# BriansIDP/espnet_slurp

Measured on AMD Instinct MI355X. Metric: utterances/sec (fbank80x1500, Conformer-12L CTC+attn), higher is better.
Workload: dtype f32; 1 GPU; C2 SLURP Conformer-medium d=256 H=4 FF=1024 12L enc / 6L dec, V=600, rel_pos=latest, ctc 0.3, lsm 0.1, dropout 0.1, SpecAug on; global_batch=384, seq_len=1500, parallelism=dp1

## Files before the change

espnet_slurp_amd/_native.py:

```python
from __future__ import annotations

import ctypes
import os

_HERE = os.path.dirname(os.path.abspath(__file__))
LIB_PATH = os.path.join(_HERE, "libespnet_mi355%s.so" % os.environ.get("ESP_LIB_VARIANT", ""))

P = ctypes.c_void_p
I = ctypes.c_int
L = ctypes.c_long
F = ctypes.c_float
U64 = ctypes.c_ulonglong

SIGNATURES = {
    "esp_last_error": [],
    "esp_abi_version": [],
    "esp_gemm_bf16": [I, I, I, I, I, I, I, P, L, L, L, P, L, L, L, P, L, L, L, P, F, F, P, I, P, F, U64, I, P, P, P, L,
                      P],
    "esp_gemm_bf16_pl": [I, I, I, I, I, I, I, P, L, L, L, P, L, L, L, P, L, L, L, P, F, F, I, P, F, U64, I, P, I,
                         L, P, L, P],
    "esp_f32_to_bf16": [P, P, L, I, L, L, I, P],
    "esp_conv2_fwd_bf16": [P, P, P, P, I, I, I, I, P, L, P],
    "esp_conv2_dgrad_bf16": [P, P, P, P, I, I, I, I, P, P, L, P],
    "esp_conv1_fwd_bf16": [P, P, P, P, P, I, I, I, I, P],
    "esp_conv2_wgrad_bf16": [P, P, P, P, I, I, I, I, P, L, P],
    "esp_gemm_f32": [I, I, I, I, I, I, I, P, L, L, L, P, L, L, L, P, L, L, L, P, F, F, P, I, P, F, U64, I, P, P,
                     P, P, P, L, P],
    "esp_gemm_f32_bp": [I, I, I, I, I, I, I, P, L, L, L, P, L, L, L, P, L, L, L, P, F, F, P, I, P, F, U64, I, P, P,
                        P, P, L, P, L, L, L, L, P],
    "esp_f32_to_planes": [P, P, L, I, L, L, L, P],
    "esp_gemm_f32_pl": [I, I, I, I, I, I, I, P, L, L, L, P, L, L, L, L, P, L, L, L, P, L, L, L, L, P, L, L, L, P, F, F,
                        P, I, P, F, U64, I, P, P, I, L, P, L, P],
    "esp_set_gemm_compute": [I],
    "esp_get_gemm_compute": [],
    "esp_f32_gemm_products": [],
    "esp_set_splitk_mode": [I],
    "esp_set_wgrad_ws": [I],
    "esp_set_fwd_ws": [I],
    "esp_get_fwd_ws_launches": [],
    "esp_act_bwd": [P, P, P, L, I, F, U64, L, P],
    "esp_scale_dropout": [P, P, L, F, F, U64, P, F, P],
    "esp_scale_dropout_planes": [P, P, L, L, I, F, F, U64, P],
    "esp_scale_by_dev": [P, L, P, P],
    "esp_embed_fwd": [P, P, P, P, I, I, I, F, F, U64, P],
    "esp_embed_bwd": [P, P, P, I, I, I, F, F, U64, P],
    "esp_specaug": [P, P, I, I, I, P, P, P, I, P, I, P],
    "esp_utterance_mvn": [P, I, I, I, P, P],
    "esp_grad_norm": [P, L, F, P, L, P, P],
    "esp_adam": [P, P, P, P, L, P, F, ctypes.c_double, ctypes.c_double, F, F, I, P],
    "esp_opt_hyper": [P, ctypes.c_double, ctypes.c_double, ctypes.c_double, ctypes.c_double, P, P],
    "esp_adam_dev": [P, P, P, P, L, P, P, ctypes.c_double, ctypes.c_double, F, F, P],
    "esp_adam_amsgrad": [P, P, P, P, P, L, P, F, ctypes.c_double, ctypes.c_double, F, F, I, P],
    "esp_adam_dev_amsgrad": [P, P, P, P, P, L, P, P, ctypes.c_double, ctypes.c_double, F, F, P],
    "esp_opt_advance": [P, P, P],
# ... 95 lines not shown
    "esp_layernorm_bwd_workspace_bytes": [I, I],
    "esp_colsum_workspace_bytes": [I, I],
    "esp_dwconv1d_wgrad_workspace_bytes": [I, I, I, I],
    "esp_ebf_merge_bwd_workspace_bytes": [I, I, I, I],
    "esp_bn_swish_fwd_workspace_bytes": [I, I],
    "esp_bn_swish_bwd_workspace_bytes": [I, I],
    "esp_conv1_wgrad_workspace_bytes": [I, I, I, I],
    "esp_conv2_dgrad_workspace_bytes": [I],
    "esp_ctc_loss_workspace_bytes": [I, I, I],
    "esp_rnnt_joint_bwd_workspace_bytes": [I, I, I, I],
    "esp_rnnt_loss_workspace_bytes": [I, I, I],
    "esp_relpos_dp_workspace_bytes": [I, I, I],
}
_RESTYPES = {"esp_last_error": ctypes.c_char_p, "esp_abi_version": I, "esp_attn_slot_check_errors": I, "esp_set_gemm_compute": I,
             "esp_get_gemm_compute": I, "esp_set_splitk_mode": I, "esp_set_wgrad_ws": I, "esp_set_fwd_ws": I, "esp_get_fwd_ws_launches": L,
             "esp_f32_gemm_products": I}
_RESTYPES.update({k: L for k in SIGNATURES if k.endswith("_workspace_bytes")})
ABI_VERSION = 42

_lib = None


def load() -> ctypes.CDLL:
    global _lib
    if _lib is not None:
        return _lib
    if not os.path.exists(LIB_PATH):
        raise RuntimeError(
            f"espnet_slurp_amd: native library not found at {LIB_PATH}; "
            "build it with `make -C espnet_slurp_amd/csrc` (no CPU fallback exists)")
# ... 31 lines not shown
```

espnet_slurp_amd/csrc/gemm.hip:

```cpp
#include <stdlib.h>

#include <algorithm>

#include "gemm_kernels.h"

using namespace espg;

namespace {

bool aligned16(const void* p) { return ((uintptr_t)p & 15) == 0; }

constexpr int RED_SLOTS = 64, RED_GROUPS = 4;
__global__ __launch_bounds__(256) void splitk_reduce4_kernel(GemmArgs g) {
  __shared__ float4 part[RED_GROUPS][RED_SLOTS];
  const long MN = (long)g.M * g.N;
  const long split_stride = MN * g.batch;
  if (g.rowsum && g.rs_work) {
    const long m = blockIdx.x * (long)blockDim.x + threadIdx.x;
    if (m < g.M) {
      float acc = 0.f;
      int s = 0;
      for (; s + 8 <= g.splits; s += 8) {
        float v[8];
#pragma unroll
// ... 71 lines not shown
  out[r] += s;
}

long g_cus = -1;
long persist_blocks(int per_cu) {
  if (g_cus < 0) {
    int dev = 0, cus = 256;
    if (hipGetDevice(&dev) == hipSuccess)
      if (hipDeviceGetAttribute(&cus, hipDeviceAttributeMultiprocessorCount, dev) != hipSuccess) cus = 256;
    g_cus = cus;
  }
  return (long)per_cu * g_cus;
}

int g_compute = 0;
int g_last_grid = 0;

int g_splitk = 0;
int splitk_mode() { return g_splitk; }

int g_wgrad_ws = 1;
int g_fwd_ws = 1;
long g_fwd_ws_launches = 0;

constexpr long kSplitkMinK = 256;
long splitk_mink() { return kSplitkMinK; }

constexpr long kSplitkTarget = 2 * 256;
constexpr long kMaxSplits = 128;
#ifndef ESP_GEMM_TILE_TIE
#define ESP_GEMM_TILE_TIE 0.95
#endif

bool launch_glds(int MA, int MB, const GemmArgs& g, int batch, hipStream_t st, const GldsArgs* tconv = nullptr) {
  const int BNT = g.bnt;
  const bool can_rs = MA == RC;
  const bool can_fwd = (MA == KC && (MB == KC || MB == RC)) || (MA == I2C_KC && MB == KC);
  const bool can_bwd = (MA == KC || MA == I2CT_KC) && MB == RC;
  const bool can_spec_fwd = MA == KC && MB == KC, can_spec_bwd = MA == KC && MB == RC;
  const bool can_brelu = (MA == KC || MA == I2C_KC) && MB == KC;
  const bool can_pspec = (MA == KC || MA == RC) && (MB == KC || MB == RC);
  if (MA == I2C_KC && (g.a.ic.C % GL_BK || g.K % GL_BK)) return false;
  if (MA == I2C_KC && 8L * g.a.ic.H * g.a.ic.W * g.a.ic.C >= (1L << 32)) return false;
  if (MB == I2C_RC) {
    const long kpix = g.bf16 == 2 ? 2L * g.K : (long)g.K;
    if (!i2c_rc_off24_ok(g.b.ic, kpix)) return false;
  }
  int kind = g.splits > 1 ? EPI_PLAIN : epi_kind_spec(g);
  if (g.cpn) {
// ... 15 lines not shown
  const int bm = g.bm == 64 || g.bm == 256 ? g.bm : BM;
  x.nty = (g.M + bm - 1) / bm;
  if (MA == I2C_KC) {
    x.c_a = make_fastdiv(g.a.ic.C);
    x.hw_a = make_fastdiv(g.a.ic.Ho * g.a.ic.Wo);
    x.wo_a = make_fastdiv(g.a.ic.Wo);
  }
  if (MB == I2C_RC) {
    x.c_b = make_fastdiv(g.b.ic.C);
    x.hw_b = make_fastdiv(g.b.ic.Ho * g.b.ic.Wo);
    x.wo_b = make_fastdiv(g.b.ic.Wo);
  }
  x.ntiles = (int)((long)x.ntx * x.nty * batch * g.splits);
  const bool rs = can_rs && g.rowsum;
  if (rs) kind = EPI_PLAIN;
  if (kind == EPI_C1FOLD && !(MA == I2CT_KC && MB == RC && BNT == 128 && bm == 128 && x.ntx <= C1NT)) return false;
  const dim3 grid((unsigned)std::min<long>(x.ntiles, persist_blocks(g.ws ? 1 : glds_occupancy_rt(BNT, kind, bm, g.bf16))));
  g_last_grid = (int)grid.x;
  x.fd_grid = make_fastdiv(grid.x);
  x.fd_ntx = make_fastdiv((uint32_t)x.ntx);
  x.fd_nty = make_fastdiv((uint32_t)x.nty);
  x.fd_splits = make_fastdiv((uint32_t)g.splits);
  x.fd_nb2 = make_fastdiv((uint32_t)g.nb2);
  const int prec = g.bf16;
  if (g.ws == 2) {
    if (rs || g.splits > 1 || MB != KC || !fwd_ws_launch(MA == I2C_KC, kind, grid, st, g, x)) return false;
    ++g_fwd_ws_launches;
    return true;
  }
  if (g.ws) return kind == EPI_PLAIN && wgrad_ws_launch(MB == I2C_RC, rs, grid, st, g, x);
  if (kind == EPI_PLAIN) return glds_launch_plain(MA, MB, BNT, prec, rs, grid, st, g, x);
  if (kind == EPI_FWD || kind == EPI_BWD) return glds_launch_epi(MA, MB, BNT, prec, kind, grid, st, g, x);
  if (kind == EPI_P0 || kind == EPI_PR || kind == EPI_SMB || kind == EPI_SMBN || kind == EPI_P0_PL)
    return glds_launch_pspec(MA, MB, BNT, prec, kind, grid, st, g, x);
  return glds_launch_spec(MA, MB, BNT, prec, kind, grid, st, g, x);
}

template <int MA, int MB>
int launch(const GemmArgs& g0, int batch, hipStream_t st, const Operand* b_fp32 = nullptr,
// ... 83 lines not shown
ESP_API int esp_f32_gemm_products(void) { return ESP_F32_SPLIT ? 6 : 1; }
ESP_API int esp_set_splitk_mode(int mode) {
  ESP_ARG_CHECK(mode == 0 || mode == 1, "esp_set_splitk_mode: mode must be 0 or 1, got %d", mode);
  const int prev = splitk_mode();
  g_splitk = mode;
  return prev;
}

ESP_API int esp_set_fwd_ws(int mode) {
  ESP_ARG_CHECK(mode >= 0 && mode <= 2, "esp_set_fwd_ws: mode must be 0, 1 or 2, got %d", mode);
  const int prev = g_fwd_ws;
  g_fwd_ws = mode;
  return prev;
}
ESP_API long esp_get_fwd_ws_launches(void) { return g_fwd_ws_launches; }

ESP_API int esp_set_wgrad_ws(int mode) {
  ESP_ARG_CHECK(mode >= 0 && mode <= 2, "esp_set_wgrad_ws: mode must be 0, 1 or 2, got %d", mode);
  const int prev = g_wgrad_ws;
  g_wgrad_ws = mode;
  return prev;
}

static int gemm_run(int mode_a, int mode_b, int M, int N, int K, int batch, int nb2, const float* A, long lda,
                    long sa1, long sa2, const float* B, long ldb, long sb1, long sb2, float* C, long ldc, long sc1,
                    long sc2, const float* bias, float alpha, float beta, const float* R, int act, float* aux,
                    float drop_p, unsigned long long seed, int bwd_act, const float* pre, float* rowsum,
                    const int* im2col_a, const int* im2col_b, float* work, long work_bytes, void* stream,
                    int prec_in, const GemmArgs* smb = nullptr, const void* b_planes = nullptr, long ldbp = 0,
                    long sbp1 = 0, long sbp2 = 0, long bps = 0, const void* a_planes = nullptr, long ldap = 0,
// ... 536 lines not shown
    hipLaunchKernelGGL(f32_to_planes_kernel, dim3((unsigned)std::min<long>((ps / 8 + 255) / 256, 8192)), dim3(256), 0,
                       st, wc_work, (uint4*)planes, 9L * D, D, (long)D, (long)D, ps, 1);
    ESP_CHECK_LAUNCH("esp_conv2_dgrad (planes)");
  }
  const int slot0[4] = {0, 4, 6, 8};
  C1Regions c1r{};
  long c1off = 0;
  for (int cls = 0; cls < 4; ++cls) {
    const int ph = cls >> 1, pw = cls & 1;
    const int Ha = (T1 - ph + 1) / 2, We = (F1 - pw + 1) / 2;
    const int nkt = ph ? 1 : 2, nkf = pw ? 1 : 2, ntap = nkt * nkf;
    GldsArgs t{};
    t.t_hw = make_fastdiv((uint32_t)(Ha * We));
    t.t_w = make_fastdiv((uint32_t)We);
    t.t_T2 = T2; t.t_F2 = F2; t.t_C = b16 ? D / 2 : D;
    for (int ti = 0; ti < ntap; ++ti) {
      const int kt = ph ? 1 : 2 * (ti / nkf), kf = pw ? 1 : 2 * (ti % nkf);
      t.t_dt[ti] = (kt - ph) / 2;
      t.t_df[ti] = (kf - pw) / 2;
    }
    t.t_zeros = zeros16;
    GemmArgs g{};
    g.M = B * Ha * We; g.N = D; g.K = b16 ? ntap * D / 2 : ntap * D; g.nb2 = 1;
    g.a = Operand{dz2, 0, 0, 0, 1, {}, 1};
    g.b = Operand{wc_work + (long)slot0[cls] * D * D, D, 0, 0, 1, {}, 1};
    g.c = dz1; g.ldc = D; g.alpha = 1.f; g.beta = 0.f;
    g.bwd_act = ACT_RELU; g.pre = z1bits ? zeros16 : z1;
    g.cm_bits = reinterpret_cast<const uint32_t*>(z1bits); g.cm_bw = D / 32;
    if (c1) {
      g.c = wc_work;
// ... 4 lines not shown
    if (bp) {
      g.b = Operand{reinterpret_cast<const float*>(planes + (long)slot0[cls] * D * D), D, 0, 0, 1, {}, 1};
      g.b.ps = ps;
      g.bf16 = 3;
    }
    if (b16) {
      g.b = Operand{reinterpret_cast<const float*>(planes + (long)slot0[cls] * D * D), D / 2, 0, 0, 1, {}, 1};
      g.bf16 = 2;
    }
    g.key = esp::rng_key_ptr();
    g.wide = 1;
    g.batch = 1; g.splits = 1; g.kchunk = g.K; g.bnt = D % 128 == 0 ? 128 : 64; g.bm = BM;
    g.cmap = 1;
    g.cm_hw = t.t_hw; g.cm_w = t.t_w;
    g.cm_T1 = T1; g.cm_F1 = F1; g.cm_ph = ph; g.cm_pw = pw;
    if (!launch_glds(I2CT_KC, RC, g, 1, st, &t)) {
      esp::set_error("esp_conv2_dgrad: no kernel for the class GEMM");
      return -1;
    }
    ESP_CHECK_LAUNCH("esp_conv2_dgrad");
    if (c1) {
      c1r.off[cls] = c1off;
      c1r.grid[cls] = g_last_grid;
      c1off += (long)g_last_grid * C1NT * 256 * 10;
    }
  }
  if (c1) {
    c1r.ncls = 4;
    float* red = c1->work + 4L * persist_blocks(4) * C1NT * 256 * 10;
    hipLaunchKernelGGL(c1fold_reduce_kernel, dim3((D / 128) * 4, C1_NCH), dim3(640), 0, st, c1->work, c1r, red);
    hipLaunchKernelGGL(c1fold_finalize_kernel, dim3((D * 10 + 255) / 256), dim3(256), 0, st, red, D, c1->dW, c1->db);
    ESP_CHECK_LAUNCH("esp_conv2_dgrad_c1fold (reduce)");
  }
  return 0;
}
```

espnet_slurp_amd/csrc/gemm_fwd_ws.hip:

```cpp
#include "gemm_kernels.h"

namespace espg {

#if ESP_FWD_WS && ESP_F32_SPLIT

namespace {

constexpr int FW_NT = 512;
constexpr int FW_PLA = FWD_WS_BM * 64, FW_PLB = FWD_WS_BN * 64;
constexpr int FW_STB = 3 * (FW_PLA + FW_PLB);

template <bool GA>
struct FwStageA {
  static constexpr int NI = FWD_WS_BM / 32;
  int rl, kq;
  uint32_t lds;
  __device__ __forceinline__ void init_lane(int pw, int lane) {
    const int qd = lane & 7;
    rl = 8 * pw + (lane >> 3);
    kq = 4 * qd;
    lds = (uint32_t)(rl * 64 + (((qd >> 1) ^ pl_kc_swz(rl)) << 4) + 8 * (qd & 1));
  }
  __device__ __forceinline__ long tap_off(const GemmArgs& g, const GldsArgs& x, int k0) const {
    const int t = (int)fdiv((uint32_t)k0, x.c_a), kt = t / 3, kf = t - 3 * kt;
    return ((long)kt * g.a.ic.W + kf) * g.a.ic.C + (k0 - t * g.a.ic.C);
  }
  __device__ __forceinline__ float4 load(const GemmArgs& g, const GldsArgs& x, int m0, int k0, long tap, int i) const {
    const int m = min(m0 + rl + 32 * i, g.M - 1);
    if constexpr (GA) {
      const float* p = g.a.p + tap + kq;
      return *reinterpret_cast<const float4*>(p + i2c_pix_off24(g.a.ic, x.hw_a, x.wo_a, (uint32_t)m));
    } else {
      return *reinterpret_cast<const float4*>(g.a.p + (long)m * g.a.ld + min(k0 + kq, g.K - 4));
    }
  }
  __device__ __forceinline__ void store(float4 w, int i, char* planes, int kv) const {
    if (!GA && kq >= kv) w = make_float4(0.f, 0.f, 0.f, 0.f);
    uint32_t h0, m0, l0, h1, m1, l1;
    esp::split3_pair<false>(w.x, w.y, h0, m0, l0);
    esp::split3_pair<false>(w.z, w.w, h1, m1, l1);
    char* d = planes + lds + i * 32 * 64;
    *reinterpret_cast<uint2*>(d) = make_uint2(h0, h1);
    *reinterpret_cast<uint2*>(d + FW_PLA) = make_uint2(m0, m1);
    *reinterpret_cast<uint2*>(d + 2 * FW_PLA) = make_uint2(l0, l1);
  }
};

template <bool GA, int EPI>
__global__ __launch_bounds__(FW_NT, 1) void gemm_fwd_ws_kernel(GemmArgs g, GldsArgs x) {
  constexpr int TM = 2, TN = 4;
  static_assert(2 * FW_STB <= 163840, "LDS");
  __shared__ __attribute__((aligned(16))) float smem[2 * FW_STB / 4];
  char* const sm = reinterpret_cast<char*>(smem);

  const int G = gridDim.x;
  int t = blockIdx.x;
  if (t >= x.ntiles) return;
  const int lane = threadIdx.x & 63;
  const int wave = __builtin_amdgcn_readfirstlane(threadIdx.x >> 6);
  const bool producer = wave >= 4;
  const int pw = wave & 3;
// ... 146 lines not shown
```

espnet_slurp_amd/csrc/gemm_kernels.h:

```cpp
#pragma once
#include <stdlib.h>

#include <algorithm>

#include <type_traits>

#include "common.h"

namespace espg {

constexpr int BM = 128, BN = 128, BK = 32, NT = 256;
#define ESP_GEMM_TICKET_BYTES 65536L
#define ESP_GEMM_TICKETS 16384L
#ifndef ESP_F32_SPLIT
#define ESP_F32_SPLIT 1
#endif
#ifndef ESP_GEMM_PIPE
#define ESP_GEMM_PIPE 1
#endif
#ifndef ESP_WGRAD_WS
#define ESP_WGRAD_WS 1
#endif
constexpr int WGRAD_WS_BM = 256;
#ifndef ESP_FWD_WS
#define ESP_FWD_WS 1
#endif
constexpr int FWD_WS_BM = 128, FWD_WS_BN = 256;

enum Mode { KC = 0, RC = 1, I2C_KC = 2, I2C_RC = 3, I2CT_KC = 4 };
enum Act { ACT_NONE = 0, ACT_RELU = 1, ACT_SWISH = 2, ACT_MUL = 3  };
constexpr int ACT_AUX_DERIV = 16;

struct FastDiv {
  uint32_t m;
  uint32_t sh;
  uint32_t d;
};
static FastDiv make_fastdiv(uint32_t d) {
  uint32_t l = 0;
  while ((1ull << l) < d) ++l;
  FastDiv f;
  f.d = d;
// ... 607 lines not shown
}

template <int EPI, int TM, int TN>
__device__ __forceinline__ void store_spec_tiles(const GemmArgs& g, int z, int mrow0, int ncol0, int lane,
                                                 f32x16 (&acc)[TM][TN]) {
  const bool full = mrow0 + TM * 32 <= g.M && ncol0 + TN * 32 <= g.N;
  if (EPI != EPI_SMB && EPI != EPI_SMBN && g.alpha == 1.0f) {
    if (full) store_spec<EPI, TM, TN, true, true>(g, z, mrow0, ncol0, lane, acc);
    else store_spec<EPI, TM, TN, false, true>(g, z, mrow0, ncol0, lane, acc);
  } else {
    if (full) store_spec<EPI, TM, TN, true>(g, z, mrow0, ncol0, lane, acc);
    else store_spec<EPI, TM, TN, false>(g, z, mrow0, ncol0, lane, acc);
  }
}
constexpr int C1NT = 4;
template <int TM, int TN>
__device__ __forceinline__ void store_c1fold(const GemmArgs& g, int mrow0, int ncol0, int lane, f32x16 (&acc)[TM][TN],
                                             float (&k)[5 * TN]) {
  const int h = lane >> 5, l32 = lane & 31, b1 = (l32 >> 1) & 1, b0 = l32 & 1;
  const uint32_t* wrow[TM][4];
  const float* xrow[TM][4];
#pragma unroll
  for (int i = 0; i < TM; ++i)
#pragma unroll
    for (int q = 0; q < 4; ++q) {
      const int m = min(mrow0 + i * 32 + 8 * q + 4 * h + (l32 & 3), g.M - 1);
      int b, t1, f1;
      row_btf(g, m, b, t1, f1);
      wrow[i][q] = g.cm_bits + (((long)b * g.cm_T1 + t1) * g.cm_F1 + f1) * g.cm_bw + (ncol0 >> 5);
      xrow[i][q] = g.c1_x + ((long)b * g.c1_T + 2 * t1) * g.c1_F + 2 * f1;
    }
#pragma unroll
  for (int j = 0; j < TN; ++j) {
    const int sh = 4 * (l32 >> 2);
// ... 12 lines not shown
        float pt[9];
#pragma unroll
        for (int kt = 0; kt < 3; ++kt)
#pragma unroll
          for (int kf = 0; kf < 3; ++kf)
            pt[kt * 3 + kf] = xp[kt * g.c1_F + kf];
#pragma unroll
        for (int e = 0; e < 4; ++e) {
          const float d = (w >> e) & 1u ? acc[i][j][4 * q + e] : 0.f;
#pragma unroll
          for (int t = 0; t < 9; ++t) a[e * 10 + t] = fmaf(d, pt[t], a[e * 10 + t]);
          a[e * 10 + 9] += d;
        }
      }
    }
    float r20[20];
#pragma unroll
    for (int u = 0; u < 20; ++u) {
      const float send = h ? a[u] : a[20 + u];
      r20[u] = (h ? a[20 + u] : a[u]) + __shfl_xor(send, 32, 64);
    }
    float r10[10];
#pragma unroll
    for (int u = 0; u < 10; ++u) {
      const float send = b1 ? r20[u] : r20[10 + u];
      r10[u] = (b1 ? r20[10 + u] : r20[u]) +
               __builtin_bit_cast(float, __builtin_amdgcn_mov_dpp(__builtin_bit_cast(int, send), 0x4E, 0xF, 0xF, false));
    }
#pragma unroll
    for (int u = 0; u < 5; ++u) {
      const float send = b0 ? r10[u] : r10[5 + u];
      k[5 * j + u] += (b0 ? r10[5 + u] : r10[u]) +
                      __builtin_bit_cast(float, __builtin_amdgcn_mov_dpp(__builtin_bit_cast(int, send), 0xB1, 0xF, 0xF, false));
    }
  }
}
template <int TM, int TN>
__device__ __forceinline__ void store_partials_wide(const GemmArgs& g, float* W, int mrow0, int ncol0, int lane,
                                                    f32x16 (&acc)[TM][TN]) {
  const int h = lane >> 5, l32 = lane & 31;
#pragma unroll
  for (int i = 0; i < TM; ++i)
#pragma unroll
    for (int j = 0; j < TN; ++j) {
      quad_transpose(acc[i][j], lane);
      const int n = ncol0 + j * 32 + 4 * (l32 >> 2);
      if (n >= g.N) continue;
#pragma unroll
      for (int q = 0; q < 4; ++q) {
// ... 1327 lines not shown
    c = cn;
  }
  if constexpr (EPI == EPI_C1FOLD) {
    c1flush();
#pragma unroll
    for (int tn = 0; tn < C1NT; ++tn)
      if (tn < x.ntx && !c1seen[tn]) {
        float* dst = c1rec(tn);
#pragma unroll
        for (int u = 0; u < 10; ++u) dst[u] = 0.f;
      }
  }
}


template <int V>
using IC = std::integral_constant<int, V>;
template <class F>
bool glds_switch(int ma, int mb, int bnt, int prec, int bm, F&& f) {
  auto tile = [&](auto A, auto B) {
    if (bnt != 64 && bnt != 128) return false;
    constexpr bool small_ok = (decltype(A)::value == KC || decltype(A)::value == RC) &&
                              (decltype(B)::value == KC || decltype(B)::value == RC);
    constexpr int MA_ = decltype(A)::value, MB_ = decltype(B)::value;
    constexpr bool planes_ok = (MB_ == KC && (MA_ == KC || MA_ == I2C_KC)) ||
                               (MB_ == RC && (MA_ == KC || MA_ == RC || MA_ == I2CT_KC));
    auto by_prec = [&](auto N, auto R) {
      if (prec == 0) {
        f(A, B, N, IC<0>{}, R);
      } else if (prec == 1) {
// ... 37 lines not shown
    case I2CT_KC * 8 + RC: return tile(IC<I2CT_KC>{}, IC<RC>{});
    default: return false;
  }
}

bool glds_launch_plain(int ma, int mb, int bnt, int prec, bool rs, dim3 grid, hipStream_t st, const GemmArgs& g,
                       const GldsArgs& x);
bool glds_launch_epi(int ma, int mb, int bnt, int prec, int epi, dim3 grid, hipStream_t st, const GemmArgs& g,
                     const GldsArgs& x);
bool glds_launch_spec(int ma, int mb, int bnt, int prec, int epi, dim3 grid, hipStream_t st, const GemmArgs& g,
                      const GldsArgs& x);
bool glds_launch_pspec(int ma, int mb, int bnt, int prec, int epi, dim3 grid, hipStream_t st, const GemmArgs& g,
                       const GldsArgs& x);
bool wgrad_ws_launch(bool gather_b, bool rs, dim3 grid, hipStream_t st, const GemmArgs& g, const GldsArgs& x);
bool fwd_ws_launch(bool gather_a, int epi, dim3 grid, hipStream_t st, const GemmArgs& g, const GldsArgs& x);
inline bool i2c_rc_off24_ok(const Im2col& ic, long kpix) {
  const long rows = kpix / ((long)ic.Ho * ic.Wo) * ic.H * ic.W;
  return rows < (1L << 24) && rows * ic.C < (1L << 32);
}
inline int glds_occupancy_rt(int bnt, int epi, int bm, int prec) {
  const int by_regs = bm == 256 ? 1 : bm == 64 ? 4 : (bnt == 64 && (epi == EPI_PLAIN || epi >= EPI_BIAS)) ? 3 : 2;
  const int by_lds = 163840 / glds_lds_bytes(bnt, bm == 64 || bm == 256 ? bm : BM, prec);
  return std::min(by_regs, by_lds);
}

}
```

espnet_slurp_amd/kernels.py:

```python
from __future__ import annotations

import math
import os
from typing import Optional, Sequence

import torch

from . import _native

KC, RC, I2C_KC, I2C_RC = 0, 1, 2, 3
ACT_NONE, ACT_RELU, ACT_SWISH = 0, 1, 2
ACT_MUL = 3
ACT_AUX_DERIV = 16


def _p(t: Optional[torch.Tensor], off: int = 0):
    if t is None:
        return None
    return t.data_ptr() + off * t.element_size()


def _st():
    return torch.cuda.current_stream().cuda_stream

# ... 711 lines not shown
    return prev


def set_fwd_ws(mode: int) -> int:
    lib = _native.load()
    prev = lib.esp_set_fwd_ws(int(mode))
    if prev < 0:
        raise _native.NativeError(f"esp_set_fwd_ws failed: {lib.esp_last_error().decode()}")
    return prev


def fwd_ws_launches() -> int:
    return int(_native.load().esp_get_fwd_ws_launches())


def get_gemm_compute() -> int:
    return _native.load().esp_get_gemm_compute()


class gemm_compute:

    def __init__(self, dtype):
        self.dtype = dtype

    def __enter__(self):
        self.prev = set_gemm_compute(self.dtype)
        return self

    def __exit__(self, *exc):
        set_gemm_compute(self.prev)
# ... 1049 lines not shown
```

include/espnet_mi355.h:

```cpp
#ifndef ESPNET_MI355_H
#define ESPNET_MI355_H
#ifdef __cplusplus
extern "C" {
#endif

const char* esp_last_error(void);
int esp_abi_version(void);

int esp_gemm_f32(int mode_a, int mode_b, int M, int N, int K, int batch, int nb2,
                 const float* A, long lda, long sa1, long sa2,
                 const float* B, long ldb, long sb1, long sb2,
                 float* C, long ldc, long sc1, long sc2,
                 const float* bias, float alpha, float beta, const float* R,
                 int act, float* aux, float drop_p, unsigned long long seed,
                 int bwd_act, const float* pre, float* rowsum,
                 const int* im2col_a, const int* im2col_b, float* work, long work_bytes,
                 void* stream);
int esp_set_gemm_compute(int dtype);
int esp_get_gemm_compute(void);
int esp_f32_gemm_products(void);
int esp_set_splitk_mode(int mode);
int esp_set_wgrad_ws(int mode);
int esp_set_fwd_ws(int mode);
long esp_get_fwd_ws_launches(void);
int esp_gemm_f32_bp(int mode_a, int mode_b, int M, int N, int K, int batch, int nb2, const float* A, long lda,
                    long sa1, long sa2, const float* B, long ldb, long sb1, long sb2, float* C, long ldc,
                    long sc1, long sc2, const float* bias, float alpha, float beta, const float* R, int act,
                    float* aux, float drop_p, unsigned long long seed, int bwd_act, const float* pre, float* rowsum,
                    const int* im2col_a, float* work, long work_bytes, const void* b_planes, long ldbp, long sbp1,
                    long sbp2, long b_pstride, void* stream);
int esp_gemm_f32_pl(int mode_a, int mode_b, int M, int N, int K, int batch, int nb2, const float* A, long lda,
                    long sa1, long sa2, const void* a_planes, long ldap, long sap1, long sap2, long a_pstride,
                    const float* B, long ldb, long sb1, long sb2, const void* b_planes, long ldbp, long sbp1,
                    long sbp2, long b_pstride, float* C, long ldc, long sc1, long sc2, const float* bias,
                    float alpha, float beta, const float* R, int act, float* aux, float drop_p,
                    unsigned long long seed, int bwd_act, const float* pre, float* rowsum, int c_nplanes,
                    long c_pstride, float* work, long work_bytes, void* stream);
int esp_f32_to_planes(const float* x, void* y, long rows, int cols, long ldx, long ldy, long pstride, void* stream);
int esp_gemm_bf16(int mode_a, int mode_b, int M, int N, int K, int batch, int nb2, const void* A, long lda,
// ... 302 lines not shown
```

Baseline: 1585 utt/s.

## Add warp-specialized producer/consumer kernel for conv2 input-gradient GEMM

Adds a persistent warp-specialized kernel for the conv2 subsampling input-gradient class GEMMs. Four producer waves gather the transposed-conv A operand and split it into bf16 planes in LDS. Four consumer waves run the MFMA triple-bf16 emulation and apply either the row-mask epilogue or the fused conv1 weight-gradient fold. It is enabled by default when enough tile rounds exist and the tap count matches an auto mask, and replaces the global last-grid variable with an explicit output parameter. The aim is to overlap the gather and plane-split latency with matrix math, at the cost of added code paths and extra LDS per block.

```diff
diff --git a/espnet_slurp_amd/_native.py b/espnet_slurp_amd/_native.py
--- a/espnet_slurp_amd/_native.py
+++ b/espnet_slurp_amd/_native.py
@@ -38,6 +38,8 @@
     "esp_set_wgrad_ws": [I],
     "esp_set_fwd_ws": [I],
     "esp_get_fwd_ws_launches": [],
+    "esp_set_dgrad_ws": [I],
+    "esp_get_dgrad_ws_launches": [],
     "esp_act_bwd": [P, P, P, L, I, F, U64, L, P],
     "esp_scale_dropout": [P, P, L, F, F, U64, P, F, P],
     "esp_scale_dropout_planes": [P, P, L, L, I, F, F, U64, P],
@@ -163,6 +165,7 @@
 }
 _RESTYPES = {"esp_last_error": ctypes.c_char_p, "esp_abi_version": I, "esp_attn_slot_check_errors": I, "esp_set_gemm_compute": I,
              "esp_get_gemm_compute": I, "esp_set_splitk_mode": I, "esp_set_wgrad_ws": I, "esp_set_fwd_ws": I, "esp_get_fwd_ws_launches": L,
+             "esp_set_dgrad_ws": I, "esp_get_dgrad_ws_launches": L,
              "esp_f32_gemm_products": I}
 _RESTYPES.update({k: L for k in SIGNATURES if k.endswith("_workspace_bytes")})
 ABI_VERSION = 42
diff --git a/espnet_slurp_amd/csrc/gemm.hip b/espnet_slurp_amd/csrc/gemm.hip
--- a/espnet_slurp_amd/csrc/gemm.hip
+++ b/espnet_slurp_amd/csrc/gemm.hip
@@ -109,7 +109,6 @@
 }
 
 int g_compute = 0;
-int g_last_grid = 0;
 
 int g_splitk = 0;
 int splitk_mode() { return g_splitk; }
@@ -117,6 +116,8 @@
 int g_wgrad_ws = 1;
 int g_fwd_ws = 1;
 long g_fwd_ws_launches = 0;
+int g_dgrad_ws = 1;
+long g_dgrad_ws_launches = 0;
 
 constexpr long kSplitkMinK = 256;
 long splitk_mink() { return kSplitkMinK; }
@@ -127,7 +128,8 @@
 #define ESP_GEMM_TILE_TIE 0.95
 #endif
 
-bool launch_glds(int MA, int MB, const GemmArgs& g, int batch, hipStream_t st, const GldsArgs* tconv = nullptr) {
+bool launch_glds(int MA, int MB, const GemmArgs& g, int batch, hipStream_t st, const GldsArgs* tconv = nullptr,
+                 int* grid_out = nullptr) {
   const int BNT = g.bnt;
   const bool can_rs = MA == RC;
   const bool can_fwd = (MA == KC && (MB == KC || MB == RC)) || (MA == I2C_KC && MB == KC);
@@ -173,15 +175,22 @@
   x.ntiles = (int)((long)x.ntx * x.nty * batch * g.splits);
   const bool rs = can_rs && g.rowsum;
   if (rs) kind = EPI_PLAIN;
-  if (kind == EPI_C1FOLD && !(MA == I2CT_KC && MB == RC && BNT == 128 && bm == 128 && x.ntx <= C1NT)) return false;
+  if (kind == EPI_C1FOLD && g.ws != 3 && !(MA == I2CT_KC && MB == RC && BNT == 128 && bm == 128 && x.ntx <= C1NT))
+    return false;
   const dim3 grid((unsigned)std::min<long>(x.ntiles, persist_blocks(g.ws ? 1 : glds_occupancy_rt(BNT, kind, bm, g.bf16))));
-  g_last_grid = (int)grid.x;
+  if (grid_out) *grid_out = (int)grid.x;
   x.fd_grid = make_fastdiv(grid.x);
   x.fd_ntx = make_fastdiv((uint32_t)x.ntx);
   x.fd_nty = make_fastdiv((uint32_t)x.nty);
   x.fd_splits = make_fastdiv((uint32_t)g.splits);
   x.fd_nb2 = make_fastdiv((uint32_t)g.nb2);
   const int prec = g.bf16;
+  if (g.ws == 3) {
+    if (rs || g.splits > 1 || batch != 1 || MA != I2CT_KC || MB != RC || prec != 3 || !dgrad_ws_launch(kind, grid, st, g, x))
+      return false;
+    ++g_dgrad_ws_launches;
+    return true;
+  }
   if (g.ws == 2) {
     if (rs || g.splits > 1 || MB != KC || !fwd_ws_launch(MA == I2C_KC, kind, grid, st, g, x)) return false;
     ++g_fwd_ws_launches;
@@ -295,6 +304,14 @@
   return prev;
 }
 ESP_API long esp_get_fwd_ws_launches(void) { return g_fwd_ws_launches; }
+
+ESP_API int esp_set_dgrad_ws(int mode) {
+  ESP_ARG_CHECK(mode >= 0 && mode <= 2, "esp_set_dgrad_ws: mode must be 0, 1 or 2, got %d", mode);
+  const int prev = g_dgrad_ws;
+  g_dgrad_ws = mode;
+  return prev;
+}
+ESP_API long esp_get_dgrad_ws_launches(void) { return g_dgrad_ws_launches; }
 
 ESP_API int esp_set_wgrad_ws(int mode) {
   ESP_ARG_CHECK(mode >= 0 && mode <= 2, "esp_set_wgrad_ws: mode must be 0, 1 or 2, got %d", mode);
@@ -861,6 +878,7 @@
     t.t_hw = make_fastdiv((uint32_t)(Ha * We));
     t.t_w = make_fastdiv((uint32_t)We);
     t.t_T2 = T2; t.t_F2 = F2; t.t_C = b16 ? D / 2 : D;
+    t.c_a = make_fastdiv((uint32_t)t.t_C);
     for (int ti = 0; ti < ntap; ++ti) {
       const int kt = ph ? 1 : 2 * (ti / nkf), kf = pw ? 1 : 2 * (ti % nkf);
       t.t_dt[ti] = (kt - ph) / 2;
@@ -895,15 +913,27 @@
     g.cmap = 1;
     g.cm_hw = t.t_hw; g.cm_w = t.t_w;
     g.cm_T1 = T1; g.cm_F1 = F1; g.cm_ph = ph; g.cm_pw = pw;
-    if (!launch_glds(I2CT_KC, RC, g, 1, st, &t)) {
+    constexpr long kDgwsMinRounds = 4;
+    constexpr unsigned kDgwsAutoTaps = 0xB;
+    if (ESP_DGRAD_WS && g_dgrad_ws && bp && z1bits && D % FWD_WS_BN == 0 && D <= 128 * C1NT && g.M < (1L << 24) &&
+        (long)B * T2 * F2 < (1L << 24) && (long)B * T2 * F2 * D < (1L << 32)) {
+      const long rounds = ((g.M + FWD_WS_BM - 1) / FWD_WS_BM) * (D / FWD_WS_BN) / persist_blocks(1);
+      if (g_dgrad_ws == 2 || (rounds >= kDgwsMinRounds && ((kDgwsAutoTaps >> (ntap - 1)) & 1u))) {
+        g.bnt = FWD_WS_BN;
+        g.bm = FWD_WS_BM;
+        g.ws = 3;
+      }
+    }
+    int grid = 0;
+    if (!launch_glds(I2CT_KC, RC, g, 1, st, &t, &grid)) {
       esp::set_error("esp_conv2_dgrad: no kernel for the class GEMM");
       return -1;
     }
     ESP_CHECK_LAUNCH("esp_conv2_dgrad");
     if (c1) {
       c1r.off[cls] = c1off;
-      c1r.grid[cls] = g_last_grid;
-      c1off += (long)g_last_grid * C1NT * 256 * 10;
+      c1r.grid[cls] = grid;
+      c1off += (long)grid * C1NT * 256 * 10;
     }
   }
   if (c1) {
diff --git a/espnet_slurp_amd/csrc/gemm_dgrad_ws.hip b/espnet_slurp_amd/csrc/gemm_dgrad_ws.hip
--- /dev/null
+++ b/espnet_slurp_amd/csrc/gemm_dgrad_ws.hip
@@ -0,0 +1,322 @@
+#include "gemm_kernels.h"
+
+namespace espg {
+
+#if ESP_DGRAD_WS && ESP_F32_SPLIT
+
+namespace {
+
+constexpr int DW_NT = 512;
+constexpr int DW_BM = FWD_WS_BM, DW_BN = FWD_WS_BN;
+constexpr int DW_PLB = DW_BN * 64;
+constexpr int DW_STB = 3 * (FW_PLA + DW_PLB);
+static_assert(2 * DW_BN / 128 <= C1NT, "EPI_C1FOLD records: 128 columns each");
+
+constexpr int DW_FOLD_PT = 12;
+constexpr int DW_FOLD_FLOATS = DW_BM * DW_FOLD_PT + DW_BM * 8;
+
+template <int TM, int TN>
+__device__ __forceinline__ void dg_fold(const GemmArgs& g, int mrow0, int rloc0, int wn, int lane, f32x16 (&acc)[TM][TN],
+                                        const float* patch, const uint32_t* mask, float (&k)[5 * TN]) {
+  const int h = lane >> 5, l32 = lane & 31;
+  const int sh = 4 * (l32 >> 2);
+#pragma unroll
+  for (int j = 0; j < TN; ++j) {
+    float a[40];
+#pragma unroll
+    for (int v = 0; v < 40; ++v) a[v] = 0.f;
+#pragma unroll
+    for (int i = 0; i < TM; ++i) {
+      quad_transpose(acc[i][j], lane);
+#pragma unroll
+      for (int q = 0; q < 4; ++q) {
+        const int r = i * 32 + 8 * q + 4 * h + (l32 & 3);
+        if (mrow0 + r >= g.M) continue;
+        const uint32_t w = mask[(rloc0 + r) * 8 + wn * TN + j] >> sh;
+        const float* xp = patch + (rloc0 + r) * DW_FOLD_PT;
+        const float4 p0 = *reinterpret_cast<const float4*>(xp), p1 = *reinterpret_cast<const float4*>(xp + 4);
+        const float pt[9] = {p0.x, p0.y, p0.z, p0.w, p1.x, p1.y, p1.z, p1.w, xp[8]};
+#pragma unroll
+        for (int e = 0; e < 4; ++e) {
+          const float d = (w >> e) & 1u ? acc[i][j][4 * q + e] : 0.f;
+#pragma unroll
+          for (int t = 0; t < 9; ++t) a[e * 10 + t] = fmaf(d, pt[t], a[e * 10 + t]);
+          a[e * 10 + 9] += d;
+        }
+      }
+    }
+    c1fold_scatter(a, lane, &k[5 * j]);
+  }
+}
+
+struct DgTap {
+  int dt, df, o0;
+};
+__device__ __forceinline__ DgTap dg_tap(const GldsArgs& x, int k0) {
+  const int t = (int)fdiv((uint32_t)k0, x.c_a);
+  return DgTap{x.t_dt[t], x.t_df[t], k0 - t * x.t_C};
+}
+__device__ __forceinline__ float4 dg_load(const GemmArgs& g, const GldsArgs& x, const FwStageA<false>& sa, int m0,
+                                          const DgTap& tp, int i, bool& in) {
+  const uint32_t m = (uint32_t)min(m0 + sa.rl + 32 * i, g.M - 1);
+  const uint32_t bb = fdiv(m, x.t_hw);
+  const uint32_t rem = m - __umul24(bb, x.t_hw.d);
+  const uint32_t aa = fdiv(rem, x.t_w);
+  const int a = (int)aa - tp.dt, e = (int)(rem - __umul24(aa, x.t_w.d)) - tp.df;
+  in = (uint32_t)a < (uint32_t)x.t_T2 && (uint32_t)e < (uint32_t)x.t_F2;
+  const uint32_t ac = (uint32_t)min(max(a, 0), x.t_T2 - 1), ec = (uint32_t)min(max(e, 0), x.t_F2 - 1);
+  const uint32_t off = __umul24(__umul24(__umul24(bb, (uint32_t)x.t_T2) + ac, (uint32_t)x.t_F2) + ec, (uint32_t)x.t_C);
+  return *reinterpret_cast<const float4*>(g.a.p + tp.o0 + sa.kq + off);
+}
+
+template <int EPI>
+__global__ __launch_bounds__(DW_NT, 1) void gemm_dgrad_ws_kernel(GemmArgs g, GldsArgs x) {
+  static_assert(EPI == EPI_RMASKMAP || EPI == EPI_C1FOLD, "the conv2 input gradient's epilogues");
+  constexpr int TM = 2, TN = 4;
+  static_assert(2 * DW_STB + 4 * (EPI == EPI_C1FOLD ? DW_FOLD_FLOATS : 0) <= 163840, "LDS");
+  __shared__ __attribute__((aligned(16))) float smem[2 * DW_STB / 4 + (EPI == EPI_C1FOLD ? DW_FOLD_FLOATS : 0)];
+  float* const fold_pt = smem + 2 * DW_STB / 4;
+  uint32_t* const fold_mk = reinterpret_cast<uint32_t*>(fold_pt + DW_BM * DW_FOLD_PT);
+  char* const sm = reinterpret_cast<char*>(smem);
+
+  const int G = gridDim.x;
+  int t = blockIdx.x;
+  if (t >= x.ntiles) {
+    if constexpr (EPI == EPI_C1FOLD) {
+      float* dst = g.c1_part + (long)blockIdx.x * C1NT * 2560;
+      for (int e = threadIdx.x; e < 2 * x.ntx * 2560; e += DW_NT) dst[e] = 0.f;
+    }
+    return;
+  }
+  const int lane = threadIdx.x & 63;
+  const int wave = __builtin_amdgcn_readfirstlane(threadIdx.x >> 6);
+  const bool producer = wave >= 4;
+  const int pw = wave & 3;
+  const int wm = pw >> 1, wn = pw & 1;
+  const int h = lane >> 5, l32 = lane & 31;
+
+  TileCoord c = tile_coord<DW_BN, DW_BM>(g, x, t, G);
+
+  FwStageA<false> sa;
+  StageP<RC, DW_BN, 4> sb;
+  constexpr int NIA = FwStageA<false>::NI;
+  float4 va[NIA];
+  uint32_t held_in = 0;
+  bool held = false, held_first = false;
+  int held_k0 = 0, held_n0 = 0;
+  int lt = t, lkt = 0;
+  TileCoord lc = c;
+  bool lok = true;
+  const uint32_t smem_lds = lds_addr(smem);
+  auto fetch = [&]() {
+    held = lok;
+    if (!lok) return;
+    const int k0 = lkt * GL_BK;
+    const DgTap tp = dg_tap(x, k0);
+    held_in = 0;
+#pragma unroll
+    for (int i = 0; i < NIA; ++i) {
+      bool in;
+      va[i] = dg_load(g, x, sa, lc.m0, tp, i, in);
+      held_in |= (uint32_t)in << i;
+    }
+    held_k0 = k0;
+    held_n0 = lc.n0;
+    held_first = lkt == 0;
+    if (++lkt == lc.nk) {
+      lt += G;
+      lkt = 0;
+      lok = lt < x.ntiles;
+      if (lok) lc = tile_coord<DW_BN, DW_BM>(g, x, lt, G);
+    }
+  };
+  auto put = [&](int stage) {
+    if (held_first) sb.init(g.b, g.b.p, g.N, held_n0, 0, pw, lane);
+    sb.issue(g.K, held_k0, smem_lds + (uint32_t)(stage * DW_STB + 3 * FW_PLA), pw);
+    char* st = sm + stage * DW_STB;
+#pragma unroll
+    for (int i = 0; i < NIA; ++i) {
+      const float4 w = (held_in >> i) & 1u ? va[i] : make_float4(0.f, 0.f, 0.f, 0.f);
+      sa.store(w, i, st, GL_BK);
+    }
+  };
+  auto publish = [&]() {
+    if (held) wait_vm_n<NIA>();
+    else wait_vm0();
+    wait_lgkm0();
+  };
+
+  float fold_x[5];
+  uint32_t fold_w[4];
+  auto fold_fetch = [&]() {
+    const int ptid = pw * 64 + lane, r = ptid >> 1, hf = ptid & 1;
+    int b, t1, f1;
+    row_btf(g, min(c.m0 + r, g.M - 1), b, t1, f1);
+    const float* xp = g.c1_x + ((long)b * g.c1_T + 2 * t1) * g.c1_F + 2 * f1;
+    const uint32_t* wp = g.cm_bits + (((long)b * g.cm_T1 + t1) * g.cm_F1 + f1) * g.cm_bw + (c.n0 >> 5) + 4 * hf;
+#pragma unroll
+    for (int u = 0; u < 4; ++u) fold_w[u] = wp[u];
+#pragma unroll
+    for (int u = 0; u < 5; ++u) {
+      const int k0 = u, k1 = min(5 + u, 8);
+      fold_x[u] = xp[hf ? (k1 / 3) * g.c1_F + k1 % 3 : (k0 / 3) * g.c1_F + k0 % 3];
+    }
+  };
+  auto fold_put = [&]() {
+    const int ptid = pw * 64 + lane, r = ptid >> 1, hf = ptid & 1;
+#pragma unroll
+    for (int u = 0; u < 4; ++u) fold_mk[r * 8 + 4 * hf + u] = fold_w[u];
+#pragma unroll
+    for (int u = 0; u < 5; ++u) fold_pt[r * DW_FOLD_PT + 5 * hf + u] = fold_x[u];
+  };
+
+  int buf = 0;
+
+  f32x16 acc[TM][TN];
+  auto slab = [&](auto role, int kt) {
+    if constexpr (decltype(role)::value) {
+      const bool fold = EPI == EPI_C1FOLD && kt == 1;
+      if (fold) fold_fetch();
+      if (held) put(buf ^ 1);
+      fetch();
+      if (fold) fold_put();
+      publish();
+    } else {
+      const char* st = sm + buf * DW_STB;
+      constexpr int PA[6] = {1, 2, 0, 1, 0, 0}, PB[6] = {1, 0, 2, 0, 1, 0};
+      auto load_b = [&](int j, int hs, bf16x8 (&bh)[3]) {
+#pragma unroll
+        for (int p = 0; p < 3; ++p)
+          bh[p] = frag_pl_rc<DW_BN>(reinterpret_cast<const float*>(st + 3 * FW_PLA + p * DW_PLB), wn * TN * 32 + j * 32,
+                                    lane, hs);
+      };
+      auto load_a = [&](int hs, bf16x8 (&ah)[TM][3]) {
+#pragma unroll
+        for (int i = 0; i < TM; ++i)
+#pragma unroll
+          for (int p = 0; p < 3; ++p)
+            ah[i][p] = frag_pl_kc(reinterpret_cast<const float*>(st + p * FW_PLA), wm * TM * 32 + i * 32 + l32, h, hs);
+      };
+      bf16x8 ah[2][TM][3], bh[2][3];
+      load_a(0, ah[0]);
+      load_b(0, 0, bh[0]);
+#pragma unroll
+      for (int u = 0; u < 2 * TN; ++u) {
+        const int hs = u / TN, j = u % TN;
+        if (u + 1 < 2 * TN) {
+          load_b((u + 1) % TN, (u + 1) / TN, bh[(u + 1) & 1]);
+          if (j + 1 == TN) load_a(1, ah[1]);
+        }
+        __builtin_amdgcn_sched_barrier(0);
+#pragma unroll
+        for (int i = 0; i < TM; ++i)
+#pragma unroll
+          for (int p = 0; p < 6; ++p)
+            acc[i][j] = __builtin_amdgcn_mfma_f32_32x32x16_bf16(ah[hs][i][PA[p]], bh[u & 1][PB[p]], acc[i][j], 0, 0, 0);
+        __builtin_amdgcn_sched_barrier(0);
+      }
+      wait_lgkm0();
+    }
+    raw_barrier();
+    buf ^= 1;
+  };
+
+  constexpr int C1K = EPI == EPI_C1FOLD ? 5 * TN : 1;
+  float c1k[C1K];
+  int c1tx = -1;
+  uint32_t c1seen = 0;
+  auto c1rec = [&](int tx, int j) {
+    return g.c1_part + ((((long)blockIdx.x * C1NT + 2 * tx + wn) * 4 + 2 * wm + (j >> 1)) * 64 + lane) * 10 + 5 * (j & 1);
+  };
+  auto c1flush = [&]() {
+    if (c1tx < 0) return;
+    const bool seen = (c1seen >> c1tx) & 1u;
+#pragma unroll
+    for (int j = 0; j < TN; ++j) {
+      float* dst = c1rec(c1tx, j);
+#pragma unroll
+      for (int u = 0; u < 5; ++u) {
+        dst[u] = seen ? dst[u] + c1k[5 * j + u] : c1k[5 * j + u];
+        c1k[5 * j + u] = 0.f;
+      }
+    }
+    c1seen |= 1u << c1tx;
+  };
+
+  auto run = [&](auto role) {
+    constexpr bool P = decltype(role)::value;
+    if constexpr (P) {
+      sa.init_lane(pw, lane);
+      fetch();
+      put(0);
+      fetch();
+      publish();
+    } else if constexpr (EPI == EPI_C1FOLD) {
+#pragma unroll
+      for (int u = 0; u < C1K; ++u) c1k[u] = 0.f;
+    }
+    raw_barrier();
+    for (;;) {
+      const int tnext = t + G;
+      const bool has_next = tnext < x.ntiles;
+      if constexpr (!P) {
+#pragma unroll
+        for (int i = 0; i < TM; ++i)
+#pragma unroll
+          for (int j = 0; j < TN; ++j)
+#pragma unroll
+            for (int r = 0; r < 16; ++r) acc[i][j][r] = 0.f;
+      }
+      for (int kt = 0; kt < c.nk; ++kt) slab(role, kt);
+      if constexpr (!P) {
+        const int mr0 = c.m0 + wm * TM * 32, nc0 = c.n0 + wn * TN * 32;
+        if constexpr (EPI == EPI_C1FOLD) {
+          if (c.tn != c1tx) {
+            c1flush();
+            c1tx = c.tn;
+          }
+          dg_fold<TM, TN>(g, mr0, wm * TM * 32, wn, lane, acc, fold_pt, fold_mk, c1k);
+        } else {
+          store_spec_tiles<EPI, TM, TN>(g, 0, mr0, nc0, lane, acc);
+        }
+      }
+      if (!has_next) break;
+      t = tnext;
+      c = tile_coord<DW_BN, DW_BM>(g, x, t, G);
+    }
+    if constexpr (!P && EPI == EPI_C1FOLD) {
+      c1flush();
+      for (int tx = 0; tx < x.ntx; ++tx)
+        if (!((c1seen >> tx) & 1u)) {
+#pragma unroll
+          for (int j = 0; j < TN; ++j) {
+            float* dst = c1rec(tx, j);
+#pragma unroll
+            for (int u = 0; u < 5; ++u) dst[u] = 0.f;
+          }
+        }
+    }
+  };
+  if (producer) run(std::true_type{});
+  else run(std::false_type{});
+}
+
+}
+
+bool dgrad_ws_launch(int epi, dim3 grid, hipStream_t st, const GemmArgs& g, const GldsArgs& x) {
+  if (g.bm != DW_BM || g.bnt != DW_BN || g.N % DW_BN || g.K % GL_BK || g.K < 2 * GL_BK || x.t_C % GL_BK || 2 * x.ntx > C1NT)
+    return false;
+  auto go = [&](auto kernel) { hipLaunchKernelGGL(kernel, grid, dim3(DW_NT), 0, st, g, x); };
+  if (epi == EPI_RMASKMAP) go(gemm_dgrad_ws_kernel<EPI_RMASKMAP>);
+  else if (epi == EPI_C1FOLD) go(gemm_dgrad_ws_kernel<EPI_C1FOLD>);
+  else return false;
+  return true;
+}
+
+#else
+
+bool dgrad_ws_launch(int, dim3, hipStream_t, const GemmArgs&, const GldsArgs&) { return false; }
+
+#endif
+
+}
diff --git a/espnet_slurp_amd/csrc/gemm_fwd_ws.hip b/espnet_slurp_amd/csrc/gemm_fwd_ws.hip
--- a/espnet_slurp_amd/csrc/gemm_fwd_ws.hip
+++ b/espnet_slurp_amd/csrc/gemm_fwd_ws.hip
@@ -7,44 +7,9 @@
 namespace {
 
 constexpr int FW_NT = 512;
-constexpr int FW_PLA = FWD_WS_BM * 64, FW_PLB = FWD_WS_BN * 64;
+constexpr int FW_PLB = FWD_WS_BN * 64;
 constexpr int FW_STB = 3 * (FW_PLA + FW_PLB);
 
-template <bool GA>
-struct FwStageA {
-  static constexpr int NI = FWD_WS_BM / 32;
-  int rl, kq;
-  uint32_t lds;
-  __device__ __forceinline__ void init_lane(int pw, int lane) {
-    const int qd = lane & 7;
-    rl = 8 * pw + (lane >> 3);
-    kq = 4 * qd;
-    lds = (uint32_t)(rl * 64 + (((qd >> 1) ^ pl_kc_swz(rl)) << 4) + 8 * (qd & 1));
-  }
-  __device__ __forceinline__ long tap_off(const GemmArgs& g, const GldsArgs& x, int k0) const {
-    const int t = (int)fdiv((uint32_t)k0, x.c_a), kt = t / 3, kf = t - 3 * kt;
-    return ((long)kt * g.a.ic.W + kf) * g.a.ic.C + (k0 - t * g.a.ic.C);
-  }
-  __device__ __forceinline__ float4 load(const GemmArgs& g, const GldsArgs& x, int m0, int k0, long tap, int i) const {
-    const int m = min(m0 + rl + 32 * i, g.M - 1);
-    if constexpr (GA) {
-      const float* p = g.a.p + tap + kq;
-      return *reinterpret_cast<const float4*>(p + i2c_pix_off24(g.a.ic, x.hw_a, x.wo_a, (uint32_t)m));
-    } else {
-      return *reinterpret_cast<const float4*>(g.a.p + (long)m * g.a.ld + min(k0 + kq, g.K - 4));
-    }
-  }
-  __device__ __forceinline__ void store(float4 w, int i, char* planes, int kv) const {
-    if (!GA && kq >= kv) w = make_float4(0.f, 0.f, 0.f, 0.f);
-    uint32_t h0, m0, l0, h1, m1, l1;
-    esp::split3_pair<false>(w.x, w.y, h0, m0, l0);
-    esp::split3_pair<false>(w.z, w.w, h1, m1, l1);
-    char* d = planes + lds + i * 32 * 64;
-    *reinterpret_cast<uint2*>(d) = make_uint2(h0, h1);
-    *reinterpret_cast<uint2*>(d + FW_PLA) = make_uint2(m0, m1);
-    *reinterpret_cast<uint2*>(d + 2 * FW_PLA) = make_uint2(l0, l1);
-  }
-};
 
 template <bool GA, int EPI>
 __global__ __launch_bounds__(FW_NT, 1) void gemm_fwd_ws_kernel(GemmArgs g, GldsArgs x) {
diff --git a/espnet_slurp_amd/csrc/gemm_kernels.h b/espnet_slurp_amd/csrc/gemm_kernels.h
--- a/espnet_slurp_amd/csrc/gemm_kernels.h
+++ b/espnet_slurp_amd/csrc/gemm_kernels.h
@@ -26,6 +26,9 @@
 #define ESP_FWD_WS 1
 #endif
 constexpr int FWD_WS_BM = 128, FWD_WS_BN = 256;
+#ifndef ESP_DGRAD_WS
+#define ESP_DGRAD_WS 1
+#endif
 
 enum Mode { KC = 0, RC = 1, I2C_KC = 2, I2C_RC = 3, I2CT_KC = 4 };
 enum Act { ACT_NONE = 0, ACT_RELU = 1, ACT_SWISH = 2, ACT_MUL = 3  };
@@ -663,10 +666,32 @@
   }
 }
 constexpr int C1NT = 4;
+__device__ __forceinline__ void c1fold_scatter(const float (&a)[40], int lane, float* k5) {
+  const int h = lane >> 5, b1 = (lane >> 1) & 1, b0 = lane & 1;
+  float r20[20];
+#pragma unroll
+  for (int u = 0; u < 20; ++u) {
+    const float send = h ? a[u] : a[20 + u];
+    r20[u] = (h ? a[20 + u] : a[u]) + __shfl_xor(send, 32, 64);
+  }
+  float r10[10];
+#pragma unroll
+  for (int u = 0; u < 10; ++u) {
+    const float send = b1 ? r20[u] : r20[10 + u];
+    r10[u] = (b1 ? r20[10 + u] : r20[u]) +
+             __builtin_bit_cast(float, __builtin_amdgcn_mov_dpp(__builtin_bit_cast(int, send), 0x4E, 0xF, 0xF, false));
+  }
+#pragma unroll
+  for (int u = 0; u < 5; ++u) {
+    const float send = b0 ? r10[u] : r10[5 + u];
+    k5[u] += (b0 ? r10[5 + u] : r10[u]) +
+             __builtin_bit_cast(float, __builtin_amdgcn_mov_dpp(__builtin_bit_cast(int, send), 0xB1, 0xF, 0xF, false));
+  }
+}
 template <int TM, int TN>
 __device__ __forceinline__ void store_c1fold(const GemmArgs& g, int mrow0, int ncol0, int lane, f32x16 (&acc)[TM][TN],
                                              float (&k)[5 * TN]) {
-  const int h = lane >> 5, l32 = lane & 31, b1 = (l32 >> 1) & 1, b0 = l32 & 1;
+  const int h = lane >> 5, l32 = lane & 31;
   const uint32_t* wrow[TM][4];
   const float* xrow[TM][4];
 #pragma unroll
@@ -709,25 +734,7 @@
         }
       }
     }
-    float r20[20];
-#pragma unroll
-    for (int u = 0; u < 20; ++u) {
-      const float send = h ? a[u] : a[20 + u];
-      r20[u] = (h ? a[20 + u] : a[u]) + __shfl_xor(send, 32, 64);
-    }
-    float r10[10];
-#pragma unroll
-    for (int u = 0; u < 10; ++u) {
-      const float send = b1 ? r20[u] : r20[10 + u];
-      r10[u] = (b1 ? r20[10 + u] : r20[u]) +
-               __builtin_bit_cast(float, __builtin_amdgcn_mov_dpp(__builtin_bit_cast(int, send), 0x4E, 0xF, 0xF, false));
-    }
-#pragma unroll
-    for (int u = 0; u < 5; ++u) {
-      const float send = b0 ? r10[u] : r10[5 + u];
-      k[5 * j + u] += (b0 ? r10[5 + u] : r10[u]) +
-                      __builtin_bit_cast(float, __builtin_amdgcn_mov_dpp(__builtin_bit_cast(int, send), 0xB1, 0xF, 0xF, false));
-    }
+    c1fold_scatter(a, lane, &k[5 * j]);
   }
 }
 template <int TM, int TN>
@@ -2085,6 +2092,43 @@
 }
 
 
+constexpr int FW_PLA = FWD_WS_BM * 64;
+template <bool GA>
+struct FwStageA {
+  static constexpr int NI = FWD_WS_BM / 32;
+  int rl, kq;
+  uint32_t lds;
+  __device__ __forceinline__ void init_lane(int pw, int lane) {
+    const int qd = lane & 7;
+    rl = 8 * pw + (lane >> 3);
+    kq = 4 * qd;
+    lds = (uint32_t)(rl * 64 + (((qd >> 1) ^ pl_kc_swz(rl)) << 4) + 8 * (qd & 1));
+  }
+  __device__ __forceinline__ long tap_off(const GemmArgs& g, const GldsArgs& x, int k0) const {
+    const int t = (int)fdiv((uint32_t)k0, x.c_a), kt = t / 3, kf = t - 3 * kt;
+    return ((long)kt * g.a.ic.W + kf) * g.a.ic.C + (k0 - t * g.a.ic.C);
+  }
+  __device__ __forceinline__ float4 load(const GemmArgs& g, const GldsArgs& x, int m0, int k0, long tap, int i) const {
+    const int m = min(m0 + rl + 32 * i, g.M - 1);
+    if constexpr (GA) {
+      const float* p = g.a.p + tap + kq;
+      return *reinterpret_cast<const float4*>(p + i2c_pix_off24(g.a.ic, x.hw_a, x.wo_a, (uint32_t)m));
+    } else {
+      return *reinterpret_cast<const float4*>(g.a.p + (long)m * g.a.ld + min(k0 + kq, g.K - 4));
+    }
+  }
+  __device__ __forceinline__ void store(float4 w, int i, char* planes, int kv) const {
+    if (!GA && kq >= kv) w = make_float4(0.f, 0.f, 0.f, 0.f);
+    uint32_t h0, m0, l0, h1, m1, l1;
+    esp::split3_pair<false>(w.x, w.y, h0, m0, l0);
+    esp::split3_pair<false>(w.z, w.w, h1, m1, l1);
+    char* d = planes + lds + i * 32 * 64;
+    *reinterpret_cast<uint2*>(d) = make_uint2(h0, h1);
+    *reinterpret_cast<uint2*>(d + FW_PLA) = make_uint2(m0, m1);
+    *reinterpret_cast<uint2*>(d + 2 * FW_PLA) = make_uint2(l0, l1);
+  }
+};
+
 template <int V>
 using IC = std::integral_constant<int, V>;
 template <class F>
@@ -2152,6 +2196,7 @@
                        const GldsArgs& x);
 bool wgrad_ws_launch(bool gather_b, bool rs, dim3 grid, hipStream_t st, const GemmArgs& g, const GldsArgs& x);
 bool fwd_ws_launch(bool gather_a, int epi, dim3 grid, hipStream_t st, const GemmArgs& g, const GldsArgs& x);
+bool dgrad_ws_launch(int epi, dim3 grid, hipStream_t st, const GemmArgs& g, const GldsArgs& x);
 inline bool i2c_rc_off24_ok(const Im2col& ic, long kpix) {
   const long rows = kpix / ((long)ic.Ho * ic.Wo) * ic.H * ic.W;
   return rows < (1L << 24) && rows * ic.C < (1L << 32);
diff --git a/espnet_slurp_amd/kernels.py b/espnet_slurp_amd/kernels.py
--- a/espnet_slurp_amd/kernels.py
+++ b/espnet_slurp_amd/kernels.py
@@ -749,6 +749,18 @@
     return int(_native.load().esp_get_fwd_ws_launches())
 
 
+def set_dgrad_ws(mode: int) -> int:
+    lib = _native.load()
+    prev = lib.esp_set_dgrad_ws(int(mode))
+    if prev < 0:
+        raise _native.NativeError(f"esp_set_dgrad_ws failed: {lib.esp_last_error().decode()}")
+    return prev
+
+
+def dgrad_ws_launches() -> int:
+    return int(_native.load().esp_get_dgrad_ws_launches())
+
+
 def get_gemm_compute() -> int:
     return _native.load().esp_get_gemm_compute()
 
diff --git a/include/espnet_mi355.h b/include/espnet_mi355.h
--- a/include/espnet_mi355.h
+++ b/include/espnet_mi355.h
@@ -23,6 +23,8 @@
 int esp_set_wgrad_ws(int mode);
 int esp_set_fwd_ws(int mode);
 long esp_get_fwd_ws_launches(void);
+int esp_set_dgrad_ws(int mode);
+long esp_get_dgrad_ws_launches(void);
 int esp_gemm_f32_bp(int mode_a, int mode_b, int M, int N, int K, int batch, int nb2, const float* A, long lda,
                     long sa1, long sa2, const float* B, long ldb, long sb1, long sb2, float* C, long ldc,
                     long sc1, long sc2, const float* bias, float alpha, float beta, const float* R, int act,
```

Result: faster. 1608 utt/s, median of 6 (+1.5%).
